# xjh19971/multi-robot-perception-gnn-1

Measured on AMD Instinct MI355X. Metric: aggregated node-features/sec (N×C×H×W elems through GCN) at 1/2/4/8 MI355X, higher is better.
Workload: dtype f32; 1 GPU; gcn_film_mean_fwd_B32_N8_complete_C512_32x32_fp32; graphs_per_rank=32, global_graphs=32, robots=8, channels=512, H=32, W=32, layers=1, parallelism=dp1 (independent graphs)

## Files before the change

include/mrp_gnn.h:

```cpp
#ifndef MRP_GNN_H
#define MRP_GNN_H

#include <stdint.h>

#ifdef __cplusplus
extern "C" {
#endif

#define MRP_MAX_NODES 16

enum mrp_graph_kind {
    MRP_GRAPH_CSR = 0,
    MRP_GRAPH_COMPLETE = 1,
    MRP_GRAPH_SIMPLE = 3
};
#define MRP_GRAPH_REGULAR(k) (((k) << 8) | 2)
#define MRP_GRAPH_IS_REGULAR(kind) (((kind) & 0xff) == 2)
#define MRP_GRAPH_REGULAR_K(kind) ((kind) >> 8)

enum mrp_agg_mode {
    MRP_AGG_FILM_MEAN = 0,
    MRP_AGG_FILM_SUM = 1,
    MRP_AGG_COPY_MEAN = 2
};
// ... 295 lines not shown
enum mrp_agg_kernel {
  MRP_AGG_KERNEL_NONE = 0,
  MRP_AGG_KERNEL_FILM_FWD = 1,
  MRP_AGG_KERNEL_FILM_FWD_REGULAR = 2,
  MRP_AGG_KERNEL_FILM_BWD_FUSED = 3,
  MRP_AGG_KERNEL_FILM_BWD_DX_GRAM = 4,
  MRP_AGG_KERNEL_FILM_BWD_REGULAR = 5,
  MRP_AGG_KERNEL_FILM_BWD_MFMA = 6
};

typedef struct mrp_agg_plan {
  int32_t kernel;
  int32_t vec;
  int32_t lpc;
  int32_t cpb;
  int32_t threads;
  int32_t psplit;
  int32_t ncb;
  int32_t pre2;
  int64_t grid;
  int64_t lds_bytes;
} mrp_agg_plan;

int mrp_film_mean_fwd_plan(int32_t dtype,
                           const void* x, int64_t x_node_stride,
                           const float* gb,
                           const int32_t* indptr, const int32_t* src, const int32_t* eid,
                           const int32_t* graph_off, int32_t num_graphs, int32_t max_nodes,
                           int32_t graph_kind, int32_t num_nodes, int32_t num_edges,
                           int32_t C, int32_t P, int32_t mode,
                           void* out, int64_t out_node_stride,
                           const mrp_agg_epilogue* epilogue,
                           mrp_agg_plan* plan);
int mrp_film_mean_bwd_plan(int32_t dtype,
                           const void* grad_out, int64_t g_node_stride,
                           const void* x, int64_t x_node_stride,
                           const float* gb,
                           const int32_t* indptr, const int32_t* src, const int32_t* eid,
                           const int32_t* graph_off, int32_t num_graphs, int32_t max_nodes,
                           int32_t graph_kind, int32_t num_nodes, int32_t num_edges,
                           int32_t C, int32_t P, int32_t mode,
                           void* grad_x, int64_t gx_node_stride,
                           const void* grad_x_base, int64_t base_node_stride,
                           float* grad_gb,
                           const mrp_agg_epilogue* epilogue,
                           mrp_agg_plan* plan);

int mrp_abi_version(void);

int mrp_stream_copy(const void* src, void* dst, int64_t bytes, void* stream);

int mrp_stream_join(void* waiter, void* signaller);

const char* mrp_error_string(int code);

#ifdef __cplusplus
}
#endif

#endif
```

multi-robot-perception-gnn-1_amd/_lib.py:

```python
from __future__ import annotations

import ctypes
import os
import threading

import torch

PKG_DIR = os.path.dirname(os.path.abspath(__file__))
LIB_PATH = os.path.join(PKG_DIR, "lib", "libmrp_gnn.so")

EXPORTED_SYMBOLS = (
    "mrp_film_mean_fwd",
    "mrp_film_mean_cat_fwd",
    "mrp_film_mean_bwd",
    "mrp_film_mean_fwd_ex",
    "mrp_film_mean_bwd_ex",
    "mrp_film_mean_fwd_t",
    "mrp_film_mean_bwd_t",
    "mrp_film_mean_fwd_plan",
    "mrp_film_mean_bwd_plan",
    "mrp_film_mean_bwd_workspace",
    "mrp_film_mean_fwd_cl",
    "mrp_film_mean_bwd_cl",
    "mrp_film_mean_bwd_cl_workspace",
    "mrp_film_max_fwd",
    "mrp_film_max_bwd",
    "mrp_compress_fwd",
    "mrp_compress_weight_transpose",
    "mrp_compress_bwd_data",
    "mrp_compress_bwd_weight_workspace",
    "mrp_compress_bwd_weight",
    "mrp_compress_split_pack_bytes",
    "mrp_compress_split_pack",
    "mrp_compress_fwd_split",
    "mrp_compress_bwd_data_split",
    "mrp_compress_bwd_weight_split_workspace",
    "mrp_compress_bwd_weight_split",
    "mrp_compress_fwd_split_p",
    "mrp_compress_bwd_data_split_p",
    "mrp_compress_bwd_weight_split_p",
    "mrp_compress_pack_t_bytes",
    "mrp_compress_pack_t",
    "mrp_compress_fwd_t",
    "mrp_compress_bwd_data_t",
    "mrp_compress_bwd_weight_t_workspace",
    "mrp_compress_bwd_weight_t",
    "mrp_compress_fwd_cl",
    "mrp_compress_bwd_data_cl",
    "mrp_compress_bwd_weight_cl_workspace",
    "mrp_compress_bwd_weight_cl",
    "mrp_compress_fwd_split_cl",
    "mrp_compress_bwd_data_split_cl",
    "mrp_compress_bwd_weight_split_cl_workspace",
    "mrp_compress_bwd_weight_split_cl",
    "mrp_edge_hidden_fwd",
    "mrp_edge_logits_fwd",
    "mrp_edge_encoder_pack_bytes",
    "mrp_edge_encoder_pack",
    "mrp_edge_encoder_fwd_split",
    "mrp_edge_encoder_fwd_split_train",
    "mrp_edge_encoder_bwd_workspace",
    "mrp_edge_encoder_bwd",
    "mrp_edge_encoder_bwd_prep",
    "mrp_edge_encoder_bwd_split_workspace",
    "mrp_edge_encoder_bwd_split",
    "mrp_edge_encoder_bwd_fused_workspace",
    "mrp_edge_encoder_bwd_fused",
    "mrp_edge_encoder_bwd_t_workspace",
    "mrp_edge_encoder_bwd_t",
    "mrp_edge_encoder_bwd_pose_workspace",
    "mrp_edge_encoder_bwd_pose",
    "mrp_frame_graph_build",
    "mrp_frame_graph_build_range",
    "mrp_frame_graph_build_range_workspace",
    "mrp_stream_copy",
    "mrp_stream_join",
    "mrp_tuning_set",
    "mrp_abi_version",
    "mrp_error_string",
)
ABI_VERSION = 22
MAX_NODES = 16
FILM_MAX_DEGREE = 16

HIP_ERROR_NOT_SUPPORTED = 801

MODE_FILM_MEAN = 0
MODE_FILM_SUM = 1
MODE_COPY_MEAN = 2
GB_LOGITS = 0x100
DTYPE_F32 = 0
DTYPE_BF16 = 1
DTYPE_F16 = 2
GRAPH_CSR = 0
GRAPH_COMPLETE = 1
GRAPH_SIMPLE = 3


MAX_REGULAR_K = 8


def graph_regular(k: int) -> int:
    return (k << 8) | 2
MODES = {"film_mean": MODE_FILM_MEAN, "film_sum": MODE_FILM_SUM, "copy_mean": MODE_COPY_MEAN}

class Epilogue(ctypes.Structure):

    _fields_ = [("agg_scale", ctypes.c_float), ("self_scale", ctypes.c_float), ("x0", ctypes.c_void_p),
                ("x0_node_stride", ctypes.c_int64), ("x0_scale", ctypes.c_float), ("xcopy", ctypes.c_void_p),
                ("xcopy_node_stride", ctypes.c_int64)]


AGG_KERNELS = ("none", "film_fwd", "film_fwd_regular", "film_bwd_fused", "film_bwd_dx_gram", "film_bwd_regular",
               "film_bwd_mfma")


class AggPlan(ctypes.Structure):

    _fields_ = [("kernel", ctypes.c_int32), ("vec", ctypes.c_int32), ("lpc", ctypes.c_int32),
                ("cpb", ctypes.c_int32), ("threads", ctypes.c_int32), ("psplit", ctypes.c_int32),
                ("ncb", ctypes.c_int32), ("pre2", ctypes.c_int32), ("grid", ctypes.c_int64),
                ("lds_bytes", ctypes.c_int64)]

    @property
    def kernel_name(self) -> str:
        return AGG_KERNELS[self.kernel]


class EpilogueCl(ctypes.Structure):

    _fields_ = Epilogue._fields_ + [("x0_pixel_stride", ctypes.c_int64), ("xcopy_pixel_stride", ctypes.c_int64)]


_lock = threading.Lock()
_lib = None

_P = ctypes.c_void_p
_I32 = ctypes.c_int32
_I64 = ctypes.c_int64


def _declare(lib: ctypes.CDLL) -> None:
    graph = [_P, _P, _P, _P, _I32, _I32, _I32, _I32, _I32, _I32, _I32, _I32]
# ... 85 lines not shown
    lib.mrp_compress_fwd_split_cl.argtypes = lib.mrp_compress_fwd_cl.argtypes[1:-1] + [_I32, _P]
    lib.mrp_compress_fwd_split_cl.restype = ctypes.c_int
    lib.mrp_compress_bwd_data_split_cl.argtypes = lib.mrp_compress_bwd_data_cl.argtypes[1:-1] + [_I32, _P]
    lib.mrp_compress_bwd_data_split_cl.restype = ctypes.c_int
    lib.mrp_compress_bwd_weight_split_cl_workspace.argtypes = [_I32, _I32, _I32]
    lib.mrp_compress_bwd_weight_split_cl_workspace.restype = ctypes.c_int64
    lib.mrp_compress_bwd_weight_split_cl.argtypes = lib.mrp_compress_bwd_weight_cl.argtypes[1:-1] + [_I32, _P]
    lib.mrp_compress_bwd_weight_split_cl.restype = ctypes.c_int
    lib.mrp_edge_hidden_fwd.argtypes = [_P, _P, _P, _I32, _I32, _P, _P]
    lib.mrp_edge_hidden_fwd.restype = ctypes.c_int
    lib.mrp_edge_logits_fwd.argtypes = [_P, _I32, _I32, _P, _P, _P, _P]
    lib.mrp_edge_logits_fwd.restype = ctypes.c_int
    lib.mrp_edge_encoder_pack_bytes.argtypes = [_I32]
    lib.mrp_edge_encoder_pack_bytes.restype = ctypes.c_int64
    lib.mrp_edge_encoder_pack.argtypes = [_P, _P, _P, _I32, _P, _P]
    lib.mrp_edge_encoder_pack.restype = ctypes.c_int
    lib.mrp_edge_encoder_fwd_split.argtypes = [_P, _P, _P, _I32, _I32, _P, _P]
    lib.mrp_edge_encoder_fwd_split.restype = ctypes.c_int
    lib.mrp_edge_encoder_fwd_split_train.argtypes = [_P, _P, _P, _I32, _I32, _P, _P, _I64, _P]
    lib.mrp_edge_encoder_fwd_split_train.restype = ctypes.c_int
    lib.mrp_edge_encoder_bwd_prep.argtypes = [_P, _I32, _I32, _P, _I64, _P]
    lib.mrp_edge_encoder_bwd_prep.restype = ctypes.c_int
    lib.mrp_edge_encoder_bwd_split_workspace.argtypes = [_I32, _I32]
    lib.mrp_edge_encoder_bwd_split_workspace.restype = ctypes.c_int64
    lib.mrp_edge_encoder_bwd_split.argtypes = [_P, _P, _P, _P, _I32, _I32, _P, _P, _P, _P, _I64, _P]
    lib.mrp_edge_encoder_bwd_split.restype = ctypes.c_int
    lib.mrp_edge_encoder_bwd_fused_workspace.argtypes = [_I32, _I32]
    lib.mrp_edge_encoder_bwd_fused_workspace.restype = ctypes.c_int64
    lib.mrp_edge_encoder_bwd_fused.argtypes = [_P, _P, _P, _P, _P, _I32, _I32, _P, _P, _P, _P, _P, _I64, _P]
    lib.mrp_edge_encoder_bwd_fused.restype = ctypes.c_int
    lib.mrp_edge_encoder_bwd_t_workspace.argtypes = [_I32, _I32]
    lib.mrp_edge_encoder_bwd_t_workspace.restype = ctypes.c_int64
    lib.mrp_edge_encoder_bwd_t.argtypes = [_P, _I64, _P, _I64, _P, _I32, _I32, _P, _P, _P, _I64, _P]
    lib.mrp_edge_encoder_bwd_t.restype = ctypes.c_int
    lib.mrp_edge_encoder_bwd_pose_workspace.argtypes = [_I32, _I32]
    lib.mrp_edge_encoder_bwd_pose_workspace.restype = ctypes.c_int64
    lib.mrp_edge_encoder_bwd_pose.argtypes = [_P, _I64, _P, _I64, _P, _I32, _I32, _P, _P, _I64, _P]
    lib.mrp_edge_encoder_bwd_pose.restype = ctypes.c_int
    lib.mrp_edge_encoder_bwd_workspace.argtypes = [_I32, _I32]
    lib.mrp_edge_encoder_bwd_workspace.restype = ctypes.c_int64
    lib.mrp_edge_encoder_bwd.argtypes = [_P, _P, _P, _P, _I32, _I32, _P, _P, _P, _P, _P]
    lib.mrp_edge_encoder_bwd.restype = ctypes.c_int
    lib.mrp_frame_graph_build.argtypes = [_P, _I32, _I32, _I32, _P, _P, _P, _P, _P, _P]
    lib.mrp_frame_graph_build.restype = ctypes.c_int
    lib.mrp_frame_graph_build_range.argtypes = [_P, _P, _I32, _I32, _I32, ctypes.c_double, _P, _P, _P, _P, _P, _P,
                                                _I64, _P]
    lib.mrp_frame_graph_build_range.restype = ctypes.c_int
    lib.mrp_frame_graph_build_range_workspace.argtypes = [_I32, _I32]
    lib.mrp_frame_graph_build_range_workspace.restype = ctypes.c_int64
    lib.mrp_stream_copy.argtypes = [_P, _P, _I64, _P]
    lib.mrp_stream_copy.restype = ctypes.c_int
    lib.mrp_stream_join.argtypes = [_P, _P]
    lib.mrp_stream_join.restype = ctypes.c_int
    lib.mrp_abi_version.argtypes = []
    lib.mrp_abi_version.restype = ctypes.c_int
    lib.mrp_error_string.argtypes = [ctypes.c_int]
    lib.mrp_error_string.restype = ctypes.c_char_p


def load_library(path: str = LIB_PATH) -> ctypes.CDLL:
    global _lib
    with _lock:
        if _lib is not None:
            return _lib
        if not os.path.isfile(path):
            raise RuntimeError(
                f"mrp_gnn: HIP library not found at {path}. Build it with "
                "`python -c 'import __graft_entry__ as g; g.build()'` (hipcc --offload-arch=gfx950). "
                "There is no CPU fallback for the aggregation kernels."
            )
        lib = ctypes.CDLL(path)
        _declare(lib)
        got = lib.mrp_abi_version()
        if got != ABI_VERSION:
            raise RuntimeError(f"mrp_gnn: ABI version mismatch: library {got}, bindings {ABI_VERSION}")
        _lib = lib
        return lib


def check(code: int, what: str) -> None:
    if code != 0:
        msg = load_library().mrp_error_string(code)
        text = msg.decode() if msg else "unknown error"
        raise RuntimeError(f"mrp_gnn: {what} failed with HIP error {code}: {text}")
```

multi-robot-perception-gnn-1_amd/build.py:

```python
from __future__ import annotations

import os
import shutil
import subprocess
import sys

PKG_DIR = os.path.dirname(os.path.abspath(__file__))
REPO = os.path.dirname(PKG_DIR)
SOURCES = [os.path.join(PKG_DIR, "csrc", f) for f in ("film_mean_bwd_1_8.hip", "film_mean_bwd_9_12.hip",
                                                    "film_mean_bwd_13_16.hip", "film_max_bwd.hip",
                                                    "film_max_bwd_bf16.hip", "film_max_bwd_f16.hip", "film_max_fwd.hip",
                                                    "film_mean_fwd.hip",
                                                    "film_mean_cl_fwd.hip", "film_mean_cl_bwd.hip",
                                                    "film_mean_bwd_half_1_8.hip", "film_mean_bwd_half_9_12.hip",
                                                    "film_mean_bwd_half_13_16.hip", "film_mean_bwd_half_mfma.hip",
                                                    "film_mean_bwd_rows_mfma.hip",
                                                    "film_mean_fwd_bf16.hip",
                                                    "film_mean_fwd_f16.hip", "film_mean_bwd.hip",
                                                    "edge_encoder.hip", "frame_graph.hip",
                                                    "compress_gemm.hip", "encoder_split.hip",
                                                    "compress_split.hip", "encoder_bwd_split.hip",
                                                    "compress_half.hip",
                                                    "compress_split_cl.hip", "compress_half_cl.hip")]
OBJ_DIR = os.path.join(PKG_DIR, "build")
HEADERS = [os.path.join(REPO, "include", "mrp_gnn.h")] + [os.path.join(PKG_DIR, "csrc", h) for h in (
    "film_mean_kernels.hpp", "film_max_kernels.hpp", "film_mean_cl_kernels.hpp", "film_mean_bwd_launch.hpp", "film_mean_fwd_launch.hpp", "fast_math.hpp", "tuning.hpp", "encoder_split.hpp",
    "compress_half_common.hpp", "gemm_common.hpp", "split_common.hpp", "split_nt.hpp")]
OUT = os.path.join(PKG_DIR, "lib", "libmrp_gnn.so")
ARCH = os.environ.get("MRP_OFFLOAD_ARCH", "gfx950")


def hipcc() -> str:
    for cand in (os.environ.get("HIPCC"), "/opt/rocm/bin/hipcc", shutil.which("hipcc")):
        if cand and os.path.exists(cand):
            return cand
    raise RuntimeError("hipcc not found (ROCm toolchain required to build the HIP library)")


def _obj(src: str) -> str:
    return os.path.join(OBJ_DIR, os.path.basename(src) + ".o")


def _stale(src: str) -> bool:
    obj = _obj(src)
    return not os.path.exists(obj) or os.path.getmtime(obj) <= max(os.path.getmtime(d) for d in [src] + HEADERS)


def needs_build(out: str = OUT) -> bool:
    if not os.path.exists(out) or any(_stale(s) for s in SOURCES):
        return True
    t = os.path.getmtime(out)
    return any(os.path.getmtime(_obj(s)) > t for s in SOURCES)


FLAGS = ["-O3", "-std=c++17", "-fPIC", "-mcode-object-version=5", "-ffp-contract=off", "-Wno-pass-failed"]
EXTRA_FLAGS = {"compress_gemm.hip": ["-fno-slp-vectorize"]}


def _compile(src: str, verbose: bool) -> str:
    obj = _obj(src)
    if not _stale(src):
        return obj
    cmd = [hipcc(), f"--offload-arch={ARCH}"] + FLAGS + EXTRA_FLAGS.get(os.path.basename(src), []) + [
        "-I", os.path.join(REPO, "include"), "-c", src,
                                                      "-o", obj + ".tmp"]
    if verbose:
        print("[mrp_gnn build]", " ".join(cmd), flush=True)
    subprocess.run(cmd, check=True)
    os.replace(obj + ".tmp", obj)
    return obj


def build(force: bool = False, verbose: bool = True) -> str:
    if not force and not needs_build():
        return OUT
    os.makedirs(os.path.dirname(OUT), exist_ok=True)
# ... 22 lines not shown
```

multi-robot-perception-gnn-1_amd/encoder.py:

```python
from __future__ import annotations

import collections
import ctypes
import os
import weakref

import torch

from . import _lib


def _ptr(t):
    return ctypes.c_void_p(t.data_ptr())


def hidden_forward(pose, w1, b1) -> torch.Tensor:
    E = pose.shape[0]
    C = w1.shape[0]
    if pose.dim() != 2 or pose.shape[1] != 9 or tuple(w1.shape) != (C, 9) or tuple(b1.shape) != (C,):
        raise ValueError("edge hidden layer shapes must be pose (E,9), w1 (C,9), b1 (C,)")
    if not pose.is_cuda:
        raise RuntimeError("mrp_gnn: the edge hidden-layer kernel runs only on the GPU; no CPU fallback")
    pose, w1, b1 = (t.contiguous().float() for t in (pose, w1, b1))
    h = torch.empty((E, C), device=pose.device, dtype=torch.float32)
# ... 69 lines not shown
    global _ENC_STREAM_MIN_WORK
    prev = _ENC_STREAM_MIN_WORK
    _ENC_STREAM_MIN_WORK = int(n)
    return prev


def _record(dev: torch.device) -> torch.cuda.Event:
    ev = torch.cuda.Event()
    ev.record(torch.cuda.current_stream(dev))
    return ev


def _track_image(img: torch.Tensor) -> None:
    iid = id(img)
    _image_ready[iid] = (weakref.ref(img, lambda _r, iid=iid: _image_ready.pop(iid, None)), _record(img.device))


def _ready_event(t: torch.Tensor) -> torch.cuda.Event:
    hit = _ready.get(id(t))
    if hit is not None and hit[0]() is t and hit[1] == t._version:
        return hit[2]
    ev = _record(t.device)
    tid = id(t)
    _ready[tid] = (weakref.ref(t, lambda _r, tid=tid: _ready.pop(tid, None)), t._version, ev)
    return ev


_ENC_PRIORITY = -1
_FAST_JOIN = True


def set_fast_join(on: bool) -> None:
    global _FAST_JOIN
    _FAST_JOIN = bool(on)


def set_encoder_stream_priority(priority: int) -> None:
    global _ENC_PRIORITY
    _ENC_PRIORITY = int(priority)
    _enc_streams.clear()
    _waited.clear()
    _recorded.clear()


def _enc_stream(dev: torch.device) -> torch.cuda.Stream:
    s = _enc_streams.get(dev.index)
    if s is None:
        lo, hi = torch.cuda.Stream.priority_range()
        prio = max(min(_ENC_PRIORITY, lo), hi)
        s = _enc_streams[dev.index] = torch.cuda.Stream(device=dev, priority=prio)
    return s


def encoder_forward_split(pose, l1: torch.nn.Linear, l2: torch.nn.Linear):
    C = l1.weight.shape[0]
    if not pose.is_cuda:
        raise RuntimeError("mrp_gnn: the edge encoder kernel runs only on the GPU; no CPU fallback")
    if tuple(l1.weight.shape) != (C, 9) or tuple(l2.weight.shape) != (2 * C, C) or l1.bias is None or C == 0:
        return None
    if C % 32 == 0 and image_supported(C):
        img = packed_weights(l1, l2)
        b2 = l2.bias.detach().contiguous().float() if l2.bias is not None else None
        b2_src = l2.bias
        Cp = C
    elif image_supported(_pad32(C)):
        rec = padded_weights(l1, l2)
        img, b2, Cp = rec.img, rec.b2, rec.Cp
        b2_src = b2
    else:
        return None
    pose_src = pose
    pose = pose.detach().contiguous().float()
    E = pose.shape[0]
    dev = pose.device
    cur = torch.cuda.current_stream(dev)
    side = _enc_begin(dev, E * C, ((pose_src, pose), (b2_src, b2)), img)
    run = side if side is not None else cur
    lib = _lib.load_library()
    with torch.cuda.device(dev), torch.cuda.stream(run):
        z = torch.empty((E, 2 * Cp), device=dev, dtype=torch.float32)
        code = lib.mrp_edge_encoder_fwd_split(_ptr(pose), _ptr(img), _ptr(b2) if b2 is not None else None, E, Cp,
                                              _ptr(z), ctypes.c_void_p(run.cuda_stream))
        if code == _lib.HIP_ERROR_NOT_SUPPORTED:
            return None
        _lib.check(code, "mrp_edge_encoder_fwd_split")
        if Cp != C:
            z = z[:, : 2 * C].contiguous()
    _enc_end(dev, side, (z,), ((pose_src, pose), (None, img), (None, b2)))
    return z


def _enc_begin(dev: torch.device, work: int, reads, img):
    if not _ENC_STREAM or work < _ENC_STREAM_MIN_WORK or torch.cuda.is_current_stream_capturing():
        PATH_COUNTS["enc_inline"] += 1
        return None
    PATH_COUNTS["enc_stream"] += 1
    side = _enc_stream(dev)
    waited = _waited.setdefault(dev.index, {})

    def wait(ev):
        if waited.get(id(ev)) is not ev:
            side.wait_event(ev)
            waited[id(ev)] = ev
            if len(waited) > 64:
                waited.clear()
                waited[id(ev)] = ev

    for src, t in reads:
        if t is None:
            continue
        same = src is not None and t.data_ptr() == src.data_ptr() and t.dtype == src.dtype
        wait(_ready_event(src) if same else _record(dev))
    hit = _image_ready.get(id(img))
    if hit is not None and hit[0]() is img:
        wait(hit[1])
    else:
        side.wait_stream(torch.cuda.current_stream(dev))
    return side


def _enc_end(dev: torch.device, side, outs, reads) -> None:
    if side is None:
        return
    cur = torch.cuda.current_stream(dev)
    if _FAST_JOIN:
        _lib.check(_lib.load_library().mrp_stream_join(ctypes.c_void_p(cur.cuda_stream),
                                                       ctypes.c_void_p(side.cuda_stream)), "mrp_stream_join")
    else:
        cur.wait_stream(side)
    for t in outs:
        t.record_stream(cur)
    rec = _recorded.setdefault(dev.index, {})
    for src, t in reads:
        if t is None:
            continue
        if src is not None and src.data_ptr() == t.data_ptr():
            t = src
        hit = rec.get(id(t))
        if hit is None or hit() is not t:
            t.record_stream(side)
            tid = id(t)
            rec[tid] = weakref.ref(t, lambda _r, tid=tid, rec=rec: rec.pop(tid, None))


def logits_forward(h, w2, b2) -> torch.Tensor:
    E, C = h.shape
    if tuple(w2.shape) != (2 * C, C) or tuple(b2.shape) != (2 * C,):
        raise ValueError("edge logits shapes must be h (E,C), w2 (2C,C), b2 (2C,)")
    if not h.is_cuda:
        raise RuntimeError("mrp_gnn: the edge logits kernel runs only on the GPU; no CPU fallback")
    h, w2, b2 = (t.contiguous().float() for t in (h, w2, b2))
    if _LOGITS_PATH == "library" or C % 32 != 0:
        return torch.addmm(b2, h, w2.t())
    z = torch.empty((E, 2 * C), device=h.device, dtype=torch.float32)
    lib = _lib.load_library()
    with torch.cuda.device(h.device):
        code = lib.mrp_edge_logits_fwd(_ptr(h), E, C, _ptr(w2), _ptr(b2), _ptr(z),
                                       ctypes.c_void_p(torch.cuda.current_stream(h.device).cuda_stream))
    _lib.check(code, "mrp_edge_logits_fwd")
    return z


_side_streams = {}


def _side_stream(dev: torch.device) -> torch.cuda.Stream:
    s = _side_streams.get(dev)
    if s is None:
        s = _side_streams[dev] = torch.cuda.Stream(device=dev)
    return s


def _grad_out(param, shape, dev):
    from .dist import grad_out_like
    g = grad_out_like(param) if param is not None else None
    return g if g is not None else torch.empty(shape, device=dev)


def encoder_backward_reductions(dz, dh, h, pose, b2=None, w1=None, b1=None):
    E, C = h.shape
    dev = h.device
    db2 = _grad_out(b2, (2 * C,), dev)
    dw1 = _grad_out(w1, (C, 9), dev)
    db1 = _grad_out(b1, (C,), dev)
    lib = _lib.load_library()
# ... 253 lines not shown
            r.b2[: 2 * C] = b2
    r.img = _pack(r.w1, r.b1, r.w2)
    _track_image(r.img)
    _padded[l2] = r
    return r


def padded_supported(E: int, C: int) -> bool:
    Ep, Cp = _pad32(E), _pad32(C)
    return E > 0 and C > 0 and Ep * 2 * Cp * 4 < (1 << 31) and image_supported(Cp)


class EdgeEncoderPaddedFunction(torch.autograd.Function):

    @staticmethod
    def forward(ctx, pose, w1, b1, w2, b2, rec):
        E, C, Cp = pose.shape[0], rec.C, rec.Cp
        Ep = _pad32(E)
        dev = pose.device
        pp = torch.zeros((Ep, 9), device=dev)
        pp[:E] = pose.detach()
        zp = torch.empty((Ep, 2 * Cp), device=dev)
        hT = torch.empty((Cp, Ep), device=dev)
        lib = _lib.load_library()
        with torch.cuda.device(dev):
            _lib.check(lib.mrp_edge_encoder_fwd_split_train(
                _ptr(pp), _ptr(rec.img), _ptr(rec.b2), Ep, Cp, _ptr(zp), _ptr(hT), Ep,
                ctypes.c_void_p(torch.cuda.current_stream(dev).cuda_stream)), "mrp_edge_encoder_fwd_split_train")
        ctx.save_for_backward(pp, hT)
        ctx.rec, ctx.E = rec, E
        ctx.has_b2 = b2 is not None
        return zp[:E, : 2 * C].contiguous()

    @staticmethod
    def backward(ctx, dz):
        pp, hT = ctx.saved_tensors
        rec, E = ctx.rec, ctx.E
        C, Cp = rec.C, rec.Cp
        dev = dz.device
        need = list(ctx.needs_input_grad[:5])
        need[4] = need[4] and ctx.has_b2
        dzp = torch.zeros((pp.shape[0], 2 * Cp), device=dev)
        dzp[:E, : 2 * C] = dz
        dpose, dw1, db1, dw2, db2 = split_backward(dzp, pp, hT, rec.w1, need,
                                                   lambda i, shape: torch.empty(shape, device=dev),
                                                   rec.w2t, rec.w2t_img)
        return (dpose[:E] if dpose is not None else None,
                dw1[:C].contiguous() if dw1 is not None else None,
                db1[:C].contiguous() if db1 is not None else None,
                dw2[: 2 * C, :C].contiguous() if dw2 is not None else None,
                db2[: 2 * C].contiguous() if db2 is not None else None, None)


def edge_logits(enc_layers: torch.nn.Sequential, pose: torch.Tensor) -> torch.Tensor:
    l1, l2 = enc_layers[0], enc_layers[2]
    if not pose.is_cuda:
        raise RuntimeError("mrp_gnn: the edge encoder kernels run only on the GPU; no CPU fallback")
    params = (pose, l1.weight, l1.bias, l2.weight, l2.bias)
    inference = not (torch.is_grad_enabled() and any(t.requires_grad for t in params))
    if _LOGITS_PATH == "split" and inference:
        z = encoder_forward_split(pose, l1, l2)
        if z is not None:
            PATH_COUNTS["split"] += 1
            return z
    C, E = l1.weight.shape[0], pose.shape[0]
    if _LOGITS_PATH == "split" and l1.bias is not None and tuple(l1.weight.shape) == (C, 9) \
            and tuple(l2.weight.shape) == (2 * C, C):
        if split_train_supported(E, C):
            PATH_COUNTS["split_train"] += 1
            return EdgeEncoderSplitFunction.apply(pose, l1.weight, l1.bias, l2.weight, l2.bias,
                                                  packed_weights(l1, l2), l2)
        if padded_supported(E, C):
            PATH_COUNTS["split_padded"] += 1
            return EdgeEncoderPaddedFunction.apply(pose, l1.weight, l1.bias, l2.weight, l2.bias,
                                                   padded_weights(l1, l2))
    PATH_COUNTS["autograd"] += 1
    return EdgeEncoderFunction.apply(*params)
```

multi-robot-perception-gnn-1_amd/models.py:

```python
from __future__ import annotations

import warnings

import torch
import torch.nn as nn

from .aggregate import (film_max, film_max_cat, film_max_mix, film_max_residual, film_mean, film_mean_cat,
                        film_mean_mix, film_mean_residual)
from .compress import compress_1x1, compress_path, film_compress, film_compress_supported
from .encoder import edge_logits


def clear_packed_weights() -> None:
    from . import compress, encoder
    compress.clear_packed_weights()
    encoder.clear_packed_weights()


class _PackedImages:

    def _apply(self, fn, *args, **kwargs):
        clear_packed_weights()
        return super()._apply(fn, *args, **kwargs)

    def load_state_dict(self, *args, **kwargs):
        out = super().load_state_dict(*args, **kwargs)
        clear_packed_weights()
        return out


class edge_encoder(_PackedImages, nn.Module):

    def __init__(self, layers_dim):
        super().__init__()
        self.layers_dim = layers_dim
        self.layers = nn.Sequential(
            nn.Linear(9, layers_dim[0]),
            nn.ReLU(),
            nn.Linear(layers_dim[0], layers_dim[1] * 2),
            nn.Sigmoid(),
        )

    def logits(self, edge: torch.Tensor) -> torch.Tensor:
        if edge.is_cuda:
            z = edge_logits(self.layers, edge)
        else:
            z = self.layers[2](self.layers[1](self.layers[0](edge.float())))
        return z.view(-1, self.layers_dim[1], 2)

    def film_params(self, edge: torch.Tensor) -> torch.Tensor:
        return torch.sigmoid(self.logits(edge))

    def forward(self, edge: torch.Tensor):
        gb = self.film_params(edge)
        return gb[:, :, 0].unsqueeze(-1).unsqueeze(-1), gb[:, :, 1].unsqueeze(-1).unsqueeze(-1)


def _opt(opt, name, default):
    return getattr(opt, name, default) if opt is not None else default


UNPICKLED_GCN_RETURN = "input"


class GCN(_PackedImages, nn.Module):

    def __init__(self, opt):
        super().__init__()
        self.opt = opt
        self.edge_encoder = edge_encoder(layers_dim=[opt.feature_dim, opt.feature_dim])
        self.gcn_return_default = "aggregate"

    def __setstate__(self, state):
        super().__setstate__(state)
        if self.__dict__.get("opt") is not None and not hasattr(self.opt, "gcn_return") \
                and "gcn_return_default" not in self.__dict__:
            self.gcn_return_default = UNPICKLED_GCN_RETURN
            if UNPICKLED_GCN_RETURN == "input":
                warnings.warn("mrp_gnn: GCN unpickled from a checkpoint without opt.gcn_return: returning the "
                              "input as the reference's GCN.forward does (models.py:226); set "
                              "opt.gcn_return='aggregate' for the message-passing result", stacklevel=2)

    def _return_mode(self) -> str:
        return _opt(self.opt, "gcn_return", self.__dict__.get("gcn_return_default", "aggregate"))

    def forward(self, g, feats: torch.Tensor = None) -> torch.Tensor:
        x = g.ndata["image"] if feats is None else feats
        if self._return_mode() == "input":
            return x
        mode = _opt(self.opt, "gcn_mode", "film_mean")
        if mode == "copy_mean":
            return film_mean(x, None, g.csr(x.device), mode)
        z = self.edge_encoder.logits(g.edata["pose"])
        if mode == "film_max":
            return film_max(x, z, g.csr(x.device), logits=True)
        return film_mean(x, z, g.csr(x.device), mode, logits=True)

    def forward_cat(self, g, feats: torch.Tensor = None) -> torch.Tensor:
        x = g.ndata["image"] if feats is None else feats
        if self._return_mode() == "input" or not x.is_cuda:
            return torch.cat((x, self(g, x)), dim=1)
        mode = _opt(self.opt, "gcn_mode", "film_mean")
        if mode == "copy_mean":
            return film_mean_cat(x, None, g.csr(x.device), mode)
        z = self.edge_encoder.logits(g.edata["pose"])
        if mode == "film_max":
            return film_max_cat(x, z, g.csr(x.device), logits=True)
        return film_mean_cat(x, z, g.csr(x.device), mode, logits=True)


    def forward_cat_compress(self, g, feats: torch.Tensor, conv: nn.Conv2d) -> torch.Tensor:
        x = feats
        if (x.is_cuda and self._return_mode() != "input" and compress_path() != "library"
                and film_compress_supported(conv, x)):
            mode = _opt(self.opt, "gcn_mode", "film_mean")
            if mode == "copy_mean":
                return film_compress(conv, x, None, g.csr(x.device), _lib_modes()[mode])
            z = self.edge_encoder.logits(g.edata["pose"])
            if mode == "film_max":
                return film_compress(conv, x, z, g.csr(x.device), _lib_logits(), reducer="max")
            return film_compress(conv, x, z, g.csr(x.device), _lib_modes()[mode] | _lib_logits())
        return compress_1x1(conv, self.forward_cat(g, x))

    def forward_residual(self, g, feats: torch.Tensor = None) -> torch.Tensor:
        x = g.ndata["image"] if feats is None else feats
        if self._return_mode() == "input" or not x.is_cuda:
            return x + self(g, x)
        mode = _opt(self.opt, "gcn_mode", "film_mean")
        if mode == "copy_mean":
            return film_mean_residual(x, None, g.csr(x.device), mode)
        z = self.edge_encoder.logits(g.edata["pose"])
        if mode == "film_max":
            return film_max_residual(x, z, g.csr(x.device), logits=True)
        return film_mean_residual(x, z, g.csr(x.device), mode, logits=True)

    def forward_mix(self, g, feats: torch.Tensor, x0: torch.Tensor, alpha: float) -> torch.Tensor:
        x = feats
        if self._return_mode() == "input" or not x.is_cuda:
            return (1.0 - alpha) * self(g, x) + alpha * x0
        mode = _opt(self.opt, "gcn_mode", "film_mean")
        if mode == "copy_mean":
            return film_mean_mix(x, None, g.csr(x.device), x0, alpha, mode)
        z = self.edge_encoder.logits(g.edata["pose"])
        if mode == "film_max":
            return film_max_mix(x, z, g.csr(x.device), x0, alpha, logits=True)
        return film_mean_mix(x, z, g.csr(x.device), x0, alpha, mode, logits=True)


def _lib_modes():
    from . import _lib
    return _lib.MODES


def _lib_logits():
    from . import _lib
    return _lib.GB_LOGITS


COMBINES = ("cat_compress", "cat", "residual", "initial_mix")


def stack_layout(opt):
    layers = int(_opt(opt, "gcn_layers", 0) or (2 if _opt(opt, "multi_gcn", False) else 1))
    combine = _opt(opt, "gcn_combine", None)
    if combine is None:
        combine = "cat_compress" if _opt(opt, "compress_gcn", False) else "cat"
    if combine not in COMBINES:
        raise ValueError(f"gcn_combine must be one of {COMBINES}, got {combine!r}")
    if layers < 1:
        raise ValueError("gcn_layers must be >= 1")
    if combine == "cat" and layers > 1:
        raise AssertionError("stacked GCN layers need compress_gcn (models.py:169)")
    return layers, combine, combine == "cat_compress"


def _build_stack(module: nn.Module, opt) -> None:
    layers, combine, convs = stack_layout(opt)
    module.gcn_layers, module.gcn_combine = layers, combine
    for i in range(1, layers + 1):
        setattr(module, f"gcn{i}", GCN(opt))
        if convs:
            setattr(module, f"conv{i}", nn.Conv2d(opt.feature_dim * 2, opt.feature_dim, kernel_size=1))


def _run_stack(module: nn.Module, g, h: torch.Tensor) -> torch.Tensor:
    h0 = h
    alpha = float(_opt(module.opt, "gcn2_alpha", 0.1))
    for i in range(1, module.gcn_layers + 1):
        gcn = getattr(module, f"gcn{i}")
        if module.gcn_combine == "cat_compress":
            h = gcn.forward_cat_compress(g, h, getattr(module, f"conv{i}"))
        elif module.gcn_combine == "cat":
            h = gcn.forward_cat(g, h)
        elif module.gcn_combine == "residual":
            h = gcn.forward_residual(g, h)
        else:
            h = gcn.forward_mix(g, h, h0, alpha)
    return h

# ... 65 lines not shown
```

Measured before the change: 735.1 billion elems/s.

## Run edge encoder into a preallocated slot ring on a side stream

Adds a native hand-off ring: a set of preallocated device buffers with per-slot completion events and a dedicated priority stream. In no-grad forward passes the edge encoder writes its logits into a ring slot on that stream, and the caller waits on the slot's done event (or skips the wait if the event already completed). Progress events are recorded only every few steps to throttle slot reuse. The aim is to remove per-call allocation and cross-stream sync cost and let the encoder overlap with other work. The price is extra bookkeeping, ctypes calls per step, and more complex stream-ordering logic.

```diff
diff --git a/include/mrp_gnn.h b/include/mrp_gnn.h
--- a/include/mrp_gnn.h
+++ b/include/mrp_gnn.h
@@ -371,6 +371,18 @@
 
 int mrp_stream_join(void* waiter, void* signaller);
 
+#define MRP_HANDOFF_SKIP_COMPLETE 1
+int mrp_encoder_handoff_create(int32_t device, int32_t priority, int32_t slots, int64_t slot_bytes, void** out);
+int mrp_encoder_handoff_destroy(void* handoff);
+int mrp_encoder_handoff_resize(void* handoff, int32_t slots, int64_t slot_bytes);
+int64_t mrp_encoder_handoff_live(void);
+int mrp_encoder_handoff_begin(void* handoff, void* caller, void* const* ready_events, int32_t num_events,
+                              void** slot, void** stream);
+int mrp_encoder_handoff_end(void* handoff, void* caller, int32_t flags, int32_t* mark);
+int mrp_encoder_handoff_mark(void* handoff, void* caller);
+int mrp_encoder_handoff_plan(int64_t step, int32_t slots, int32_t* slot, int64_t* wait_progress,
+                             int64_t* record_progress);
+
 const char* mrp_error_string(int code);
 
 #ifdef __cplusplus
diff --git a/multi-robot-perception-gnn-1_amd/_lib.py b/multi-robot-perception-gnn-1_amd/_lib.py
--- a/multi-robot-perception-gnn-1_amd/_lib.py
+++ b/multi-robot-perception-gnn-1_amd/_lib.py
@@ -75,6 +75,14 @@
     "mrp_frame_graph_build_range_workspace",
     "mrp_stream_copy",
     "mrp_stream_join",
+    "mrp_encoder_handoff_create",
+    "mrp_encoder_handoff_destroy",
+    "mrp_encoder_handoff_resize",
+    "mrp_encoder_handoff_live",
+    "mrp_encoder_handoff_begin",
+    "mrp_encoder_handoff_end",
+    "mrp_encoder_handoff_mark",
+    "mrp_encoder_handoff_plan",
     "mrp_tuning_set",
     "mrp_abi_version",
     "mrp_error_string",
@@ -89,6 +97,7 @@
 MODE_FILM_SUM = 1
 MODE_COPY_MEAN = 2
 GB_LOGITS = 0x100
+HANDOFF_SKIP_COMPLETE = 1
 DTYPE_F32 = 0
 DTYPE_BF16 = 1
 DTYPE_F16 = 2
@@ -280,6 +289,24 @@
     lib.mrp_stream_copy.restype = ctypes.c_int
     lib.mrp_stream_join.argtypes = [_P, _P]
     lib.mrp_stream_join.restype = ctypes.c_int
+    pp = ctypes.POINTER(ctypes.c_void_p)
+    lib.mrp_encoder_handoff_create.argtypes = [_I32, _I32, _I32, _I64, pp]
+    lib.mrp_encoder_handoff_create.restype = ctypes.c_int
+    lib.mrp_encoder_handoff_destroy.argtypes = [_P]
+    lib.mrp_encoder_handoff_destroy.restype = ctypes.c_int
+    lib.mrp_encoder_handoff_resize.argtypes = [_P, _I32, _I64]
+    lib.mrp_encoder_handoff_resize.restype = ctypes.c_int
+    lib.mrp_encoder_handoff_live.argtypes = []
+    lib.mrp_encoder_handoff_live.restype = ctypes.c_int64
+    lib.mrp_encoder_handoff_begin.argtypes = [_P, _P, pp, _I32, pp, pp]
+    lib.mrp_encoder_handoff_begin.restype = ctypes.c_int
+    lib.mrp_encoder_handoff_end.argtypes = [_P, _P, _I32, ctypes.POINTER(_I32)]
+    lib.mrp_encoder_handoff_end.restype = ctypes.c_int
+    lib.mrp_encoder_handoff_mark.argtypes = [_P, _P]
+    lib.mrp_encoder_handoff_mark.restype = ctypes.c_int
+    lib.mrp_encoder_handoff_plan.argtypes = [_I64, _I32, ctypes.POINTER(_I32), ctypes.POINTER(_I64),
+                                             ctypes.POINTER(_I64)]
+    lib.mrp_encoder_handoff_plan.restype = ctypes.c_int
     lib.mrp_abi_version.argtypes = []
     lib.mrp_abi_version.restype = ctypes.c_int
     lib.mrp_error_string.argtypes = [ctypes.c_int]
diff --git a/multi-robot-perception-gnn-1_amd/build.py b/multi-robot-perception-gnn-1_amd/build.py
--- a/multi-robot-perception-gnn-1_amd/build.py
+++ b/multi-robot-perception-gnn-1_amd/build.py
@@ -21,7 +21,8 @@
                                                     "compress_gemm.hip", "encoder_split.hip",
                                                     "compress_split.hip", "encoder_bwd_split.hip",
                                                     "compress_half.hip",
-                                                    "compress_split_cl.hip", "compress_half_cl.hip")]
+                                                    "compress_split_cl.hip", "compress_half_cl.hip",
+                                                    "encoder_handoff.hip")]
 OBJ_DIR = os.path.join(PKG_DIR, "build")
 HEADERS = [os.path.join(REPO, "include", "mrp_gnn.h")] + [os.path.join(PKG_DIR, "csrc", h) for h in (
     "film_mean_kernels.hpp", "film_max_kernels.hpp", "film_mean_cl_kernels.hpp", "film_mean_bwd_launch.hpp", "film_mean_fwd_launch.hpp", "fast_math.hpp", "tuning.hpp", "encoder_split.hpp",
diff --git a/multi-robot-perception-gnn-1_amd/csrc/encoder_handoff.hip b/multi-robot-perception-gnn-1_amd/csrc/encoder_handoff.hip
--- /dev/null
+++ b/multi-robot-perception-gnn-1_amd/csrc/encoder_handoff.hip
@@ -0,0 +1,267 @@
+#include <hip/hip_runtime.h>
+
+#include <atomic>
+#include <cstdint>
+#include <mutex>
+#include <vector>
+
+#include "mrp_gnn.h"
+
+namespace {
+
+std::atomic<int64_t> g_live{0};
+
+constexpr int kMaxSlots = 64;
+constexpr hipError_t kOk = hipSuccess;
+
+inline int progress_stride(int slots) { return slots / 2 > 1 ? slots / 2 : 1; }
+
+struct Handoff {
+  std::mutex mu;
+  int device = 0;
+  int slots = 0;
+  int stride = 1;
+  int64_t slot_bytes = 0;
+  hipStream_t stream = nullptr;
+  std::vector<void*> buf;
+  std::vector<hipEvent_t> done;
+  std::vector<hipEvent_t> progress;
+  hipEvent_t resync = nullptr;
+  int64_t step = 0;
+  int64_t covered = -1;
+  int64_t recorded = -1;
+  int64_t pending_mark = -1;
+  bool open = false;
+  hipStream_t last_caller = nullptr;
+  bool have_caller = false;
+};
+
+struct DeviceGuard {
+  int prev = -1;
+  bool switched = false;
+  hipError_t enter(int device) {
+    hipError_t e = hipGetDevice(&prev);
+    if (e != kOk) return e;
+    if (prev != device) {
+      e = hipSetDevice(device);
+      switched = e == kOk;
+    }
+    return e;
+  }
+  ~DeviceGuard() {
+    if (switched) (void)hipSetDevice(prev);
+  }
+};
+
+void release_slots(Handoff* h) {
+  for (hipEvent_t e : h->done)
+    if (e) (void)hipEventDestroy(e);
+  for (hipEvent_t e : h->progress)
+    if (e) (void)hipEventDestroy(e);
+  for (void* p : h->buf)
+    if (p) (void)hipFree(p);
+  h->done.clear();
+  h->progress.clear();
+  h->buf.clear();
+}
+
+void release(Handoff* h) {
+  release_slots(h);
+  if (h->resync) (void)hipEventDestroy(h->resync);
+  if (h->stream) (void)hipStreamDestroy(h->stream);
+  delete h;
+}
+
+hipError_t new_event(hipEvent_t* ev) {
+  return hipEventCreateWithFlags(ev, hipEventDisableTiming | hipEventReleaseToDevice);
+}
+
+hipError_t make_slots(Handoff* h, int slots, int64_t slot_bytes) {
+  h->slots = slots;
+  h->stride = progress_stride(slots);
+  h->slot_bytes = slot_bytes;
+  h->buf.assign((size_t)slots, nullptr);
+  h->done.assign((size_t)slots, nullptr);
+  h->progress.assign((size_t)(slots / h->stride + 2), nullptr);
+  h->step = 0;
+  h->covered = h->recorded = h->pending_mark = -1;
+  h->open = false;
+  hipError_t e = kOk;
+  for (size_t i = 0; e == kOk && i < h->buf.size(); ++i) e = hipMalloc(&h->buf[i], (size_t)slot_bytes);
+  for (size_t i = 0; e == kOk && i < h->done.size(); ++i) e = new_event(&h->done[i]);
+  for (size_t i = 0; e == kOk && i < h->progress.size(); ++i) e = new_event(&h->progress[i]);
+  return e;
+}
+
+hipError_t resynchronise(Handoff* h) {
+  if (h->have_caller) {
+    hipError_t e = hipEventRecord(h->resync, h->last_caller);
+    if (e == kOk) e = hipStreamWaitEvent(h->stream, h->resync, 0);
+    if (e != kOk) {
+      (void)hipGetLastError();
+      e = hipDeviceSynchronize();
+      if (e != kOk) return e;
+    }
+  }
+  h->covered = h->step - 1;
+  h->pending_mark = -1;
+  return kOk;
+}
+
+hipError_t record_progress(Handoff* h, hipStream_t caller) {
+  const int64_t p = h->pending_mark;
+  if (p < 0) return kOk;
+  const hipError_t e = hipEventRecord(h->progress[(size_t)(p % (int64_t)h->progress.size())], caller);
+  if (e != kOk) return e;
+  h->recorded = p;
+  h->pending_mark = -1;
+  return kOk;
+}
+
+}
+
+extern "C" {
+
+int mrp_encoder_handoff_plan(int64_t step, int32_t slots, int32_t* slot, int64_t* wait_progress,
+                             int64_t* record_progress_index) {
+  if (step < 0 || slots < 1 || slots > kMaxSlots) return hipErrorInvalidValue;
+  const int64_t H = progress_stride(slots);
+  if (slot) *slot = (int32_t)(step % slots);
+  if (wait_progress) *wait_progress = step >= slots ? (step - slots) / H : -1;
+  if (record_progress_index) *record_progress_index = (step + 1) % H == 0 ? (step + 1) / H - 1 : -1;
+  return hipSuccess;
+}
+
+int mrp_encoder_handoff_create(int32_t device, int32_t priority, int32_t slots, int64_t slot_bytes, void** out) {
+  if (!out) return hipErrorInvalidValue;
+  *out = nullptr;
+  if (device < 0 || slots < 1 || slots > kMaxSlots || slot_bytes <= 0) return hipErrorInvalidValue;
+  DeviceGuard guard;
+  hipError_t e = guard.enter(device);
+  if (e != kOk) return e;
+  int lo = 0, hi = 0;
+  e = hipDeviceGetStreamPriorityRange(&lo, &hi);
+  if (e != kOk) return e;
+  if (priority > lo) priority = lo;
+  if (priority < hi) priority = hi;
+  Handoff* h = new Handoff;
+  h->device = device;
+  e = hipStreamCreateWithPriority(&h->stream, hipStreamNonBlocking, priority);
+  if (e == kOk) e = make_slots(h, slots, slot_bytes);
+  if (e == kOk) e = new_event(&h->resync);
+  if (e != kOk) {
+    release(h);
+    return e;
+  }
+  g_live.fetch_add(1);
+  *out = h;
+  return hipSuccess;
+}
+
+int mrp_encoder_handoff_destroy(void* handle) {
+  if (!handle) return hipSuccess;
+  Handoff* h = static_cast<Handoff*>(handle);
+  DeviceGuard guard;
+  hipError_t e = guard.enter(h->device);
+  if (e != kOk) return e;
+  e = hipDeviceSynchronize();
+  release(h);
+  g_live.fetch_sub(1);
+  return e;
+}
+
+int mrp_encoder_handoff_resize(void* handle, int32_t slots, int64_t slot_bytes) {
+  if (!handle || slots < 1 || slots > kMaxSlots || slot_bytes <= 0) return hipErrorInvalidValue;
+  Handoff* h = static_cast<Handoff*>(handle);
+  std::lock_guard<std::mutex> lock(h->mu);
+  if (h->open) return hipErrorInvalidValue;
+  DeviceGuard guard;
+  hipError_t e = guard.enter(h->device);
+  if (e != kOk) return e;
+  e = hipDeviceSynchronize();
+  if (e != kOk) return e;
+  release_slots(h);
+  e = make_slots(h, slots, slot_bytes);
+  if (e != kOk) release_slots(h);
+  return e;
+}
+
+int64_t mrp_encoder_handoff_live(void) { return g_live.load(); }
+
+int mrp_encoder_handoff_begin(void* handle, void* caller, void* const* ready_events, int32_t num_events,
+                              void** slot, void** stream) {
+  if (!handle || !slot || !stream || num_events < 0 || (num_events > 0 && !ready_events))
+    return hipErrorInvalidValue;
+  Handoff* h = static_cast<Handoff*>(handle);
+  std::lock_guard<std::mutex> lock(h->mu);
+  if (h->open || h->buf.empty()) return hipErrorInvalidValue;
+  hipStream_t cur = static_cast<hipStream_t>(caller);
+  hipError_t e = kOk;
+  if (h->have_caller && cur != h->last_caller) {
+    e = resynchronise(h);
+  } else if (h->pending_mark >= 0) {
+    e = record_progress(h, h->last_caller);
+  }
+  if (e != kOk) return e;
+  const int64_t need = h->step - h->slots;
+  if (need > h->covered) {
+    const int64_t p = need / h->stride;
+    if (p <= h->recorded) {
+      e = hipStreamWaitEvent(h->stream, h->progress[(size_t)(p % (int64_t)h->progress.size())], 0);
+      if (e != kOk) return e;
+      h->covered = (p + 1) * h->stride - 1;
+    } else {
+      e = resynchronise(h);
+      if (e != kOk) return e;
+    }
+  }
+  for (int32_t i = 0; i < num_events; ++i) {
+    if (!ready_events[i]) return hipErrorInvalidValue;
+    e = hipStreamWaitEvent(h->stream, static_cast<hipEvent_t>(ready_events[i]), 0);
+    if (e != kOk) return e;
+  }
+  *slot = h->buf[(size_t)(h->step % h->slots)];
+  *stream = h->stream;
+  h->open = true;
+  return hipSuccess;
+}
+
+int mrp_encoder_handoff_end(void* handle, void* caller, int32_t flags, int32_t* mark) {
+  if (!handle || (flags & ~MRP_HANDOFF_SKIP_COMPLETE) != 0) return hipErrorInvalidValue;
+  Handoff* h = static_cast<Handoff*>(handle);
+  std::lock_guard<std::mutex> lock(h->mu);
+  if (!h->open) return hipErrorInvalidValue;
+  hipStream_t cur = static_cast<hipStream_t>(caller);
+  hipEvent_t done = h->done[(size_t)(h->step % h->slots)];
+  hipError_t e = hipEventRecord(done, h->stream);
+  if (e != kOk) return e;
+  bool wait = true;
+  if (flags & MRP_HANDOFF_SKIP_COMPLETE) {
+    const hipError_t q = hipEventQuery(done);
+    if (q == kOk) wait = false;
+    else if (q == hipErrorNotReady) (void)hipGetLastError();
+    else return q;
+  }
+  if (wait) {
+    e = hipStreamWaitEvent(cur, done, 0);
+    if (e != kOk) return e;
+  }
+  h->open = false;
+  h->last_caller = cur;
+  h->have_caller = true;
+  h->pending_mark = (h->step + 1) % h->stride == 0 ? (h->step + 1) / h->stride - 1 : -1;
+  if (mark) *mark = h->pending_mark >= 0 ? 1 : 0;
+  ++h->step;
+  return hipSuccess;
+}
+
+int mrp_encoder_handoff_mark(void* handle, void* caller) {
+  if (!handle) return hipErrorInvalidValue;
+  Handoff* h = static_cast<Handoff*>(handle);
+  std::lock_guard<std::mutex> lock(h->mu);
+  if (h->open) return hipErrorInvalidValue;
+  if (h->have_caller && static_cast<hipStream_t>(caller) != h->last_caller) return hipErrorInvalidValue;
+  return record_progress(h, static_cast<hipStream_t>(caller));
+}
+
+}
diff --git a/multi-robot-perception-gnn-1_amd/encoder.py b/multi-robot-perception-gnn-1_amd/encoder.py
--- a/multi-robot-perception-gnn-1_amd/encoder.py
+++ b/multi-robot-perception-gnn-1_amd/encoder.py
@@ -145,7 +145,124 @@
     return s
 
 
-def encoder_forward_split(pose, l1: torch.nn.Linear, l2: torch.nn.Linear):
+_RING_SLOTS = int(os.environ.get("MRP_ENCODER_RING", "8"))
+RING_CAP_BYTES = 64 << 20
+_RING_CAP = RING_CAP_BYTES
+_RING_MIN_SLOT = 1 << 20
+_RING_SLOT_GRAIN = 1 << 16
+_RING_SKIP_COMPLETE = os.environ.get("MRP_ENCODER_RING_SKIP", "1") != "0"
+_rings = {}
+
+
+def set_encoder_ring_slots(n: int) -> int:
+    global _RING_SLOTS
+    prev = _RING_SLOTS
+    n = int(n)
+    if n < 0 or n > 64:
+        raise ValueError("the hand-off ring holds 0 to 64 buffers")
+    _RING_SLOTS = n
+    return prev
+
+
+def _set_ring_cap(nbytes: int) -> int:
+    global _RING_CAP
+    prev = _RING_CAP
+    _RING_CAP = int(nbytes)
+    return prev
+
+
+def _set_ring_skip_complete(on: bool) -> bool:
+    global _RING_SKIP_COMPLETE
+    prev = _RING_SKIP_COMPLETE
+    _RING_SKIP_COMPLETE = bool(on)
+    return prev
+
+
+def ring_slot_bytes(E: int, C: int, slots: int, cap: int = None):
+    cap = _RING_CAP if cap is None else cap
+    need = E * 2 * C * 4
+    if slots < 2 or need <= 0:
+        return None
+    size = max(-(-need // _RING_SLOT_GRAIN) * _RING_SLOT_GRAIN, _RING_MIN_SLOT)
+    if size * slots > cap:
+        size = -(-need // 256) * 256
+    return size if size * slots <= cap else None
+
+
+class _SlotMemory:
+
+    def __init__(self, ptr: int, nfloats: int):
+        self.__cuda_array_interface__ = {"shape": (nfloats,), "typestr": "<f4", "data": (ptr, False),
+                                         "strides": None, "version": 2}
+
+
+class _Ring:
+
+    def __init__(self, dev: torch.device, priority: int, slots: int, slot_bytes: int):
+        self.dev, self.priority, self.slots, self.slot_bytes = dev, priority, slots, slot_bytes
+        self.key = ("ring", dev.index, priority)
+        self.lib = _lib.load_library()
+        h = ctypes.c_void_p()
+        _lib.check(self.lib.mrp_encoder_handoff_create(dev.index, priority, slots, slot_bytes, ctypes.byref(h)),
+                   "mrp_encoder_handoff_create")
+        self.handle = h
+        self.stream = None
+        self.flat = {}
+
+    def resize(self, slots: int, slot_bytes: int) -> None:
+        self.flat.clear()
+        self.slots = self.slot_bytes = 0
+        _lib.check(self.lib.mrp_encoder_handoff_resize(self.handle, slots, slot_bytes), "mrp_encoder_handoff_resize")
+        self.slots, self.slot_bytes = slots, slot_bytes
+
+    def begin(self, cur, events):
+        n = len(events)
+        arr = (ctypes.c_void_p * max(n, 1))(*[ev.cuda_event for ev in events])
+        slot, stream = ctypes.c_void_p(), ctypes.c_void_p()
+        _lib.check(self.lib.mrp_encoder_handoff_begin(self.handle, ctypes.c_void_p(cur.cuda_stream), arr, n,
+                                                      ctypes.byref(slot), ctypes.byref(stream)),
+                   "mrp_encoder_handoff_begin")
+        if self.stream is None:
+            self.stream = torch.cuda.ExternalStream(stream.value, device=self.dev)
+        flat = self.flat.get(slot.value)
+        if flat is None:
+            flat = self.flat[slot.value] = torch.as_tensor(_SlotMemory(slot.value, self.slot_bytes // 4),
+                                                           device=self.dev)
+            assert flat.data_ptr() == slot.value and flat.dtype == torch.float32
+        return flat, stream
+
+    def end(self, cur) -> bool:
+        mark = ctypes.c_int32(0)
+        _lib.check(self.lib.mrp_encoder_handoff_end(self.handle, ctypes.c_void_p(cur.cuda_stream),
+                                                    1 if _RING_SKIP_COMPLETE else 0, ctypes.byref(mark)),
+                   "mrp_encoder_handoff_end")
+        return bool(mark.value)
+
+    def mark(self, cur) -> None:
+        _lib.check(self.lib.mrp_encoder_handoff_mark(self.handle, ctypes.c_void_p(cur.cuda_stream)),
+                   "mrp_encoder_handoff_mark")
+
+
+def _ring_for(dev: torch.device, E: int, C: int):
+    if (_RING_SLOTS < 2 or not _ENC_STREAM or E * C < _ENC_STREAM_MIN_WORK or E == 0
+            or torch.cuda.is_current_stream_capturing()):
+        return None
+    size = ring_slot_bytes(E, C, _RING_SLOTS)
+    if size is None:
+        return None
+    lo, hi = torch.cuda.Stream.priority_range()
+    prio = max(min(_ENC_PRIORITY, lo), hi)
+    key = (dev.index, prio)
+    ring = _rings.get(key)
+    if ring is not None and (ring.slots != _RING_SLOTS or ring.slot_bytes < E * 2 * C * 4
+                             or ring.slots * ring.slot_bytes > _RING_CAP):
+        ring.resize(_RING_SLOTS, size)
+    if ring is None:
+        ring = _rings[key] = _Ring(dev, prio, _RING_SLOTS, size)
+    return ring
+
+
+def encoder_forward_split(pose, l1: torch.nn.Linear, l2: torch.nn.Linear, ring: bool = False):
     C = l1.weight.shape[0]
     if not pose.is_cuda:
         raise RuntimeError("mrp_gnn: the edge encoder kernel runs only on the GPU; no CPU fallback")
@@ -167,9 +284,22 @@
     E = pose.shape[0]
     dev = pose.device
     cur = torch.cuda.current_stream(dev)
+    lib = _lib.load_library()
+    rg = _ring_for(dev, E, C) if ring and Cp == C else None
+    if rg is not None:
+        PATH_COUNTS["enc_stream"] += 1
+        PATH_COUNTS["enc_ring"] += 1
+        with torch.cuda.device(dev):
+            flat, stream = rg.begin(cur, _new_waits(rg.key, dev, ((pose_src, pose), (b2_src, b2)), img))
+            z = flat[: E * 2 * C].view(E, 2 * C)
+            code = lib.mrp_edge_encoder_fwd_split(_ptr(pose), _ptr(img), _ptr(b2) if b2 is not None else None, E, C,
+                                                  _ptr(z), stream)
+            mark = rg.end(cur)
+        _lib.check(code, "mrp_edge_encoder_fwd_split")
+        _record_inputs(rg.key, rg.stream, ((pose_src, pose), (None, img), (None, b2)))
+        return z, ((lambda: rg.mark(cur)) if mark else None)
     side = _enc_begin(dev, E * C, ((pose_src, pose), (b2_src, b2)), img)
     run = side if side is not None else cur
-    lib = _lib.load_library()
     with torch.cuda.device(dev), torch.cuda.stream(run):
         z = torch.empty((E, 2 * Cp), device=dev, dtype=torch.float32)
         code = lib.mrp_edge_encoder_fwd_split(_ptr(pose), _ptr(img), _ptr(b2) if b2 is not None else None, E, Cp,
@@ -180,20 +310,16 @@
         if Cp != C:
             z = z[:, : 2 * C].contiguous()
     _enc_end(dev, side, (z,), ((pose_src, pose), (None, img), (None, b2)))
-    return z
-
-
-def _enc_begin(dev: torch.device, work: int, reads, img):
-    if not _ENC_STREAM or work < _ENC_STREAM_MIN_WORK or torch.cuda.is_current_stream_capturing():
-        PATH_COUNTS["enc_inline"] += 1
-        return None
-    PATH_COUNTS["enc_stream"] += 1
-    side = _enc_stream(dev)
-    waited = _waited.setdefault(dev.index, {})
+    return (z, None) if ring else z
+
+
+def _new_waits(key, dev: torch.device, reads, img) -> list:
+    waited = _waited.setdefault(key, {})
+    out = []
 
     def wait(ev):
         if waited.get(id(ev)) is not ev:
-            side.wait_event(ev)
+            out.append(ev)
             waited[id(ev)] = ev
             if len(waited) > 64:
                 waited.clear()
@@ -208,7 +334,18 @@
     if hit is not None and hit[0]() is img:
         wait(hit[1])
     else:
-        side.wait_stream(torch.cuda.current_stream(dev))
+        out.append(_record(dev))
+    return out
+
+
+def _enc_begin(dev: torch.device, work: int, reads, img):
+    if not _ENC_STREAM or work < _ENC_STREAM_MIN_WORK or torch.cuda.is_current_stream_capturing():
+        PATH_COUNTS["enc_inline"] += 1
+        return None
+    PATH_COUNTS["enc_stream"] += 1
+    side = _enc_stream(dev)
+    for ev in _new_waits(dev.index, dev, reads, img):
+        side.wait_event(ev)
     return side
 
 
@@ -223,7 +360,11 @@
         cur.wait_stream(side)
     for t in outs:
         t.record_stream(cur)
-    rec = _recorded.setdefault(dev.index, {})
+    _record_inputs(dev.index, side, reads)
+
+
+def _record_inputs(key, side, reads) -> None:
+    rec = _recorded.setdefault(key, {})
     for src, t in reads:
         if t is None:
             continue
@@ -583,6 +724,16 @@
                 db2[: 2 * C].contiguous() if db2 is not None else None, None)
 
 
+def edge_logits_handoff(enc_layers: torch.nn.Sequential, pose: torch.Tensor):
+    l1, l2 = enc_layers[0], enc_layers[2]
+    if _LOGITS_PATH == "split" and pose.is_cuda and not torch.is_grad_enabled():
+        hit = encoder_forward_split(pose, l1, l2, ring=True)
+        if hit is not None:
+            PATH_COUNTS["split"] += 1
+            return hit
+    return edge_logits(enc_layers, pose), None
+
+
 def edge_logits(enc_layers: torch.nn.Sequential, pose: torch.Tensor) -> torch.Tensor:
     l1, l2 = enc_layers[0], enc_layers[2]
     if not pose.is_cuda:
diff --git a/multi-robot-perception-gnn-1_amd/models.py b/multi-robot-perception-gnn-1_amd/models.py
--- a/multi-robot-perception-gnn-1_amd/models.py
+++ b/multi-robot-perception-gnn-1_amd/models.py
@@ -8,7 +8,7 @@
 from .aggregate import (film_max, film_max_cat, film_max_mix, film_max_residual, film_mean, film_mean_cat,
                         film_mean_mix, film_mean_residual)
 from .compress import compress_1x1, compress_path, film_compress, film_compress_supported
-from .encoder import edge_logits
+from .encoder import edge_logits, edge_logits_handoff
 
 
 def clear_packed_weights() -> None:
@@ -47,6 +47,12 @@
         else:
             z = self.layers[2](self.layers[1](self.layers[0](edge.float())))
         return z.view(-1, self.layers_dim[1], 2)
+
+    def logits_handoff(self, edge: torch.Tensor):
+        if edge.is_cuda and not torch.is_grad_enabled():
+            z, done = edge_logits_handoff(self.layers, edge)
+            return z.view(-1, self.layers_dim[1], 2), done
+        return self.logits(edge), None
 
     def film_params(self, edge: torch.Tensor) -> torch.Tensor:
         return torch.sigmoid(self.logits(edge))
@@ -91,10 +97,17 @@
         mode = _opt(self.opt, "gcn_mode", "film_mean")
         if mode == "copy_mean":
             return film_mean(x, None, g.csr(x.device), mode)
-        z = self.edge_encoder.logits(g.edata["pose"])
-        if mode == "film_max":
-            return film_max(x, z, g.csr(x.device), logits=True)
-        return film_mean(x, z, g.csr(x.device), mode, logits=True)
+        if mode == "film_max":
+            return self._fed(g, lambda z: film_max(x, z, g.csr(x.device), logits=True))
+        return self._fed(g, lambda z: film_mean(x, z, g.csr(x.device), mode, logits=True))
+
+    def _fed(self, g, aggregate):
+        z, done = self.edge_encoder.logits_handoff(g.edata["pose"])
+        try:
+            return aggregate(z)
+        finally:
+            if done is not None:
+                done()
 
     def forward_cat(self, g, feats: torch.Tensor = None) -> torch.Tensor:
         x = g.ndata["image"] if feats is None else feats
@@ -103,10 +116,9 @@
         mode = _opt(self.opt, "gcn_mode", "film_mean")
         if mode == "copy_mean":
             return film_mean_cat(x, None, g.csr(x.device), mode)
-        z = self.edge_encoder.logits(g.edata["pose"])
-        if mode == "film_max":
-            return film_max_cat(x, z, g.csr(x.device), logits=True)
-        return film_mean_cat(x, z, g.csr(x.device), mode, logits=True)
+        if mode == "film_max":
+            return self._fed(g, lambda z: film_max_cat(x, z, g.csr(x.device), logits=True))
+        return self._fed(g, lambda z: film_mean_cat(x, z, g.csr(x.device), mode, logits=True))
 
 
     def forward_cat_compress(self, g, feats: torch.Tensor, conv: nn.Conv2d) -> torch.Tensor:
@@ -116,10 +128,11 @@
             mode = _opt(self.opt, "gcn_mode", "film_mean")
             if mode == "copy_mean":
                 return film_compress(conv, x, None, g.csr(x.device), _lib_modes()[mode])
-            z = self.edge_encoder.logits(g.edata["pose"])
             if mode == "film_max":
-                return film_compress(conv, x, z, g.csr(x.device), _lib_logits(), reducer="max")
-            return film_compress(conv, x, z, g.csr(x.device), _lib_modes()[mode] | _lib_logits())
+                return self._fed(g, lambda z: film_compress(conv, x, z, g.csr(x.device), _lib_logits(),
+                                                            reducer="max"))
+            return self._fed(g, lambda z: film_compress(conv, x, z, g.csr(x.device),
+                                                        _lib_modes()[mode] | _lib_logits()))
         return compress_1x1(conv, self.forward_cat(g, x))
 
     def forward_residual(self, g, feats: torch.Tensor = None) -> torch.Tensor:
@@ -129,10 +142,9 @@
         mode = _opt(self.opt, "gcn_mode", "film_mean")
         if mode == "copy_mean":
             return film_mean_residual(x, None, g.csr(x.device), mode)
-        z = self.edge_encoder.logits(g.edata["pose"])
-        if mode == "film_max":
-            return film_max_residual(x, z, g.csr(x.device), logits=True)
-        return film_mean_residual(x, z, g.csr(x.device), mode, logits=True)
+        if mode == "film_max":
+            return self._fed(g, lambda z: film_max_residual(x, z, g.csr(x.device), logits=True))
+        return self._fed(g, lambda z: film_mean_residual(x, z, g.csr(x.device), mode, logits=True))
 
     def forward_mix(self, g, feats: torch.Tensor, x0: torch.Tensor, alpha: float) -> torch.Tensor:
         x = feats
@@ -141,10 +153,9 @@
         mode = _opt(self.opt, "gcn_mode", "film_mean")
         if mode == "copy_mean":
             return film_mean_mix(x, None, g.csr(x.device), x0, alpha, mode)
-        z = self.edge_encoder.logits(g.edata["pose"])
-        if mode == "film_max":
-            return film_max_mix(x, z, g.csr(x.device), x0, alpha, logits=True)
-        return film_mean_mix(x, z, g.csr(x.device), x0, alpha, mode, logits=True)
+        if mode == "film_max":
+            return self._fed(g, lambda z: film_max_mix(x, z, g.csr(x.device), x0, alpha, logits=True))
+        return self._fed(g, lambda z: film_mean_mix(x, z, g.csr(x.device), x0, alpha, mode, logits=True))
 
 
 def _lib_modes():
```

After: 743.5 billion elems/s, median of 6. No clear change (+1.1%).
